# microsoft/fadtk

Hardware: NVIDIA H100
Metric: audio_seconds_embedded_per_second (higher is better)
Workload: dtype f16

## Files before the change

fadtk_b200/csrc/conv_gemm.cuh:

```cuda
#pragma once
#include "sm90.cuh"

namespace fad {

struct ConvGemmParams {
    int taps;
    int cblks;
    int box_w, box_h, box_n;
    int tiles_w, tiles_h;
    int img_groups;
    int n_tiles;
    int H, W, NB, Cout;
    int lo_adds;
    int ld_out, n_valid;
    int relu, pool;
    const float* bias;
    __half* out;
    float* out_f32;
    float* resid;
    int resid_C, resid_res, resid_shift;
};

__device__ __forceinline__ long long window_row_to_token(long long o, int res, int shift) {
    const int lg_nw = 28 - __clz(res);
// ... 2 lines not shown
    const long long wi = o >> 6;
    const int wx = (int)wi & (nw - 1);
    const int wy = (int)(wi >> lg_nw) & (nw - 1);
    const long long b = wi >> (2 * lg_nw);
    int y = wy * 8 + (in >> 3) + shift, xx = wx * 8 + (in & 7) + shift;
    if (y >= res) y -= res;
    if (xx >= res) xx -= res;
    return (b * res + y) * res + xx;
}

constexpr int kTileM = 128;
constexpr int kBlockK = 64;
constexpr int kConvGemmThreads = 512;
constexpr int kConsumers = 2;
constexpr int kConsumerRegs = 168;
constexpr int kEpiRegs = 136;
constexpr int kClusterCtas = 2;
constexpr int kChunkSteps = 8;
constexpr float kAccumShrinkPerElement = 1.06e-9f;
constexpr uint32_t kABytes = kTileM * kBlockK * 2;
constexpr uint32_t kEpiRowBytes = 128 * 4;
constexpr uint32_t kEpiBytes = 64 * kEpiRowBytes;
constexpr uint32_t kBiasBytes = 128 * 4;
static_assert(40 + kEpiRegs + kConsumers * kConsumerRegs <= 65536 / 128, "register file over-subscribed");
static_assert(kConsumerRegs > 65536 / kConvGemmThreads, "the consumers raise their register count (setmaxnreg.inc)");

template <int N_TILE, int WMODE>
__host__ __device__ constexpr uint32_t conv_gemm_stage_bytes() {
    return kABytes + (WMODE == 1 ? 2 : 1) * N_TILE * kBlockK * 2;
}

template <int N_TILE, int STAGES, int WMODE>
__host__ __device__ constexpr uint32_t conv_gemm_smem_bytes() {
    return STAGES * conv_gemm_stage_bytes<N_TILE, WMODE>() + 1024  + 256
         + kConsumers * kEpiBytes + 4 * kBiasBytes;
}

__device__ __forceinline__ uint32_t pack_half2(float a, float b) {
    __half2 h = __floats2half2_rn(a, b);
    return *reinterpret_cast<uint32_t*>(&h);
}
template <int N>
__device__ __forceinline__ void gelu_erf_n(float* x) {
    float z[N], q[N];
#pragma unroll
    for (int i = 0; i < N; ++i) { z[i] = fminf(fabsf(x[i]) * 0.70710678118654752f, 4.3f); q[i] = 1.04899843e-04f; }
    constexpr float kQ[6] = {-4.92790774e-04f, -2.22368206e-03f, 2.93586859e-02f, -1.48908889e-01f, -9.18342944e-01f,
                             -1.62791250e+00f};
#pragma unroll
    for (int t = 0; t < 6; ++t) {
#pragma unroll
        for (int i = 0; i < N; ++i) q[i] = fmaf(q[i], z[i], kQ[t]);
    }
#pragma unroll
    for (int i = 0; i < N; ++i) asm("ex2.approx.ftz.f32 %0, %1;" : "=f"(q[i]) : "f"(q[i] * z[i]));
#pragma unroll
    for (int i = 0; i < N; ++i) x[i] = 0.5f * x[i] * (1.0f + copysignf(1.0f - q[i], x[i]));
}
__device__ __forceinline__ float gelu_erf(float x) {
    gelu_erf_n<1>(&x);
    return x;
}

template <int N>
__device__ __forceinline__ void elu_ex2_n(float* x) {
    float e[N], t[N];
#pragma unroll
    for (int i = 0; i < N; ++i) asm("ex2.approx.ftz.f32 %0, %1;" : "=f"(e[i]) : "f"(fminf(x[i], 0.f) * 1.4426950408889634f));
#pragma unroll
    for (int i = 0; i < N; ++i) t[i] = x[i] * fmaf(x[i], fmaf(x[i], fmaf(x[i], 4.16666667e-2f, 1.66666667e-1f), 0.5f), 1.0f);
#pragma unroll
    for (int i = 0; i < N; ++i) x[i] = x[i] > 0.f ? x[i] : (x[i] > -0.0625f ? t[i] : e[i] - 1.0f);
}

__device__ __forceinline__ uint32_t hmax2_u32(uint32_t a, uint32_t b) {
    __half2 r = __hmax2(*reinterpret_cast<__half2*>(&a), *reinterpret_cast<__half2*>(&b));
    return *reinterpret_cast<uint32_t*>(&r);
}

template <int N_TILE, int STAGES, int WMODE>
__global__ void __launch_bounds__(kConvGemmThreads, 1)
conv_gemm_kernel(const __grid_constant__ CUtensorMap map_x,
                 const __grid_constant__ CUtensorMap map_w,
                 const ConvGemmParams p)
{
    using namespace sm90;
    static_assert(N_TILE == 128, "one m64n128 accumulator per consumer warpgroup");
    static_assert(WMODE == 0 || WMODE == 1, "WMODE 0: fp16 weights, 1: fp16 hi/lo pair");
    static_assert(kClusterCtas == 2, "the work units below are M-tile pairs");
    constexpr bool SPLIT_W = WMODE == 1;
    constexpr uint32_t kStageBytes = conv_gemm_stage_bytes<N_TILE, WMODE>();
    constexpr int kBRows = (SPLIT_W ? 2 : 1) * N_TILE;
    constexpr int kGroups = N_TILE / 32;

    extern __shared__ uint8_t smem_raw[];
    uint8_t* smem = reinterpret_cast<uint8_t*>((reinterpret_cast<uintptr_t>(smem_raw) + 1023) & ~uintptr_t(1023));
    uint64_t* bars = reinterpret_cast<uint64_t*>(smem + STAGES * kStageBytes);
    uint64_t* full = bars;
    uint64_t* empty = bars + STAGES;
    uint64_t* epi_full = bars + 2 * STAGES;
    uint64_t* epi_empty = bars + 2 * STAGES + kConsumers;
    static_assert((2 * STAGES + 2 * kConsumers) * 8 <= 256, "barriers");
    uint8_t* epi = smem + STAGES * kStageBytes + 256;

    const int warp = threadIdx.x >> 5;
    const int lane = threadIdx.x & 31;
    const int ksteps = p.taps * p.cblks;
    const int n_chunks = (ksteps + kChunkSteps - 1) / kChunkSteps;
    const int chunk_len = (ksteps + n_chunks - 1) / n_chunks;
    const int m_tiles = p.img_groups * p.tiles_h * p.tiles_w;
    const int n_clusters = (int)gridDim.x / kClusterCtas;
    const int total_units = (m_tiles + 1) / 2 * p.n_tiles;

    if (warp == 0 && lane == 0) {
        tma_prefetch_desc(&map_x);
        tma_prefetch_desc(&map_w);
    }
    if (warp == 1 && lane == 0) {
        for (int s = 0; s < STAGES; ++s) { mbar_init(&full[s], 1); mbar_init(&empty[s], kClusterCtas * kConsumers * 4); }
        for (int c = 0; c < kConsumers; ++c) { mbar_init(&epi_full[c], 128); mbar_init(&epi_empty[c], 64); }
        mbar_fence_init();
    }
    cluster_sync();

    if (warp < 4) {
        setmaxnreg_dec<40>();
        if (warp == 0 && elect_one()) {
            const int rank = (int)cluster_ctarank();
            const int cluster = (int)cluster_index();
            constexpr int kHalfRows = kBRows / kClusterCtas;
            uint8_t* const w_half = smem + kABytes + rank * kHalfRows * 128;
            int s = 0; uint32_t ph = 0;
            for (int unit = cluster; unit < total_units; unit += n_clusters) {
                const int nt = unit % p.n_tiles;
                const int m = min(2 * (unit / p.n_tiles) + rank, m_tiles - 1);
                const int w0 = (m % p.tiles_w) * p.box_w;
                const int h0 = ((m / p.tiles_w) % p.tiles_h) * p.box_h;
                const int n0 = (m / (p.tiles_w * p.tiles_h)) * p.box_n;
                for (int ks = 0; ks < ksteps; ++ks) {
                    const int tap = ks / p.cblks;
                    const int cb = ks - tap * p.cblks;
                    int dh = 0, dw = 0;
                    if (p.taps == 9) { dh = tap / 3 - 1; dw = tap % 3 - 1; }
                    mbar_wait(&empty[s], ph ^ 1);
                    uint8_t* st = smem + s * kStageBytes;
                    mbar_expect_tx(&full[s], kStageBytes);
                    tma_load_4d(st, &map_x, &full[s], cb * kBlockK, w0 + dw, h0 + dh, n0);
                    tma_load_2d_multicast(w_half + s * kStageBytes, &map_w, &full[s], ks * kBlockK,
                                          nt * kBRows + rank * kHalfRows, (1u << kClusterCtas) - 1);
                    if (++s == STAGES) { s = 0; ph ^= 1; }
                }
            }
        }
    } else if (warp < 4 + 4 * kConsumers) {
        setmaxnreg_inc<kConsumerRegs>();
        const int cluster = (int)cluster_index();
        const int c = (warp >> 2) - 1;
        const int wq = warp & 3;
        const uint32_t epi_base = smem_u32(epi) + c * kEpiBytes;
        int s = 0; uint32_t ph = 0, eph = 0;
        auto release = [&](int st_) {
            __syncwarp();
            if (lane == 0) {
#pragma unroll
                for (int cta = 0; cta < kClusterCtas; ++cta) mbar_arrive_cluster(&empty[st_], cta);
            }
        };

        for (int unit = cluster; unit < total_units; unit += n_clusters) {
            float sum[64], acc[64];
#pragma unroll
            for (int i = 0; i < 64; ++i) sum[i] = 0.f;
            for (int ks0 = 0; ks0 < ksteps; ks0 += chunk_len) {
                const int ks1 = min(ks0 + chunk_len, ksteps);
                const float unshrink = kAccumShrinkPerElement * (float)((ks1 - ks0) * kBlockK * (SPLIT_W && p.lo_adds ? 2 : 1));
                int prev_s = -1;
                for (int ks = ks0; ks < ks1; ++ks) {
                    mbar_wait(&full[s], ph);
                    const uint32_t a_addr = smem_u32(smem + s * kStageBytes);
                    const uint64_t a_desc = kmajor_sw128_desc(a_addr + c * 64 * 128);
                    const uint64_t b_desc = kmajor_sw128_desc(a_addr + kABytes);
                    wgmma_fence();
#pragma unroll
                    for (int k = 0; k < kBlockK / 16; ++k) {
                        wgmma_m64n128k16_f16<0, 0>(acc, a_desc + 2 * k, b_desc + 2 * k, (ks > ks0) || (k > 0));
                        if (SPLIT_W)
                            wgmma_m64n128k16_f16<0, 0>(acc, a_desc + 2 * k, b_desc + 2 * k + (N_TILE * 128 / 16), 1);
                    }
                    wgmma_commit();
                    wgmma_wait<1>();
                    if (prev_s >= 0) release(prev_s);
                    prev_s = s;
                    if (++s == STAGES) { s = 0; ph ^= 1; }
                }
                wgmma_wait<0>();
                fence_regs(acc);
                release(prev_s);
#pragma unroll
                for (int i = 0; i < 64; ++i) sum[i] += fmaf(acc[i], unshrink, acc[i]);
            }

            mbar_wait(&epi_empty[c], eph ^ 1);
            const int fr = wq * 16 + (lane >> 2);
            const uint32_t x = ((lane & 3) >> 1) ^ (fr & 7);
            const uint32_t row_base = epi_base + fr * kEpiRowBytes + (lane & 1) * 8;
#pragma unroll
            for (int jl = 0; jl < 4; ++jl) {
                const uint32_t a = row_base + (((2 * jl) ^ x) << 4);
#pragma unroll
                for (int jh = 0; jh < 4; ++jh) {
#pragma unroll
                    for (int i = 0; i < 2; ++i) {
                        const int j = 4 * jh + jl;
                        sts64(a + i * 8 * kEpiRowBytes + jh * 128, sum[4 * j + 2 * i], sum[4 * j + 2 * i + 1]);
                    }
                }
            }
            mbar_arrive(&epi_full[c]);
            eph ^= 1;
        }
    } else {
        if constexpr (kEpiRegs > 65536 / kConvGemmThreads) setmaxnreg_inc<kEpiRegs>();
        else setmaxnreg_dec<kEpiRegs>();
        const int rank = (int)cluster_ctarank();
        const int cluster = (int)cluster_index();
        const int e = warp - 4 - 4 * kConsumers;
        const int c = e >> 1;
        const int rr = (e & 1) * 32 + lane;
        const int r = c * 64 + rr;
        const int bw = p.box_w, bh = p.box_h;
        const int pw = r % bw;
        const int phh = (r / bw) % bh;
        const int pn = r / (bw * bh);
        const uint32_t wrows = smem_u32(epi) + c * kEpiBytes + (e & 1) * 32 * kEpiRowBytes;
        const uint32_t row_mine = wrows + lane * kEpiRowBytes;
        const uint32_t bias_s = smem_u32(epi) + kConsumers * kEpiBytes + e * kBiasBytes;
        const int sw = lane & 7;
        const int cq = lane & 7, rq = lane >> 3;
        uint32_t eph = 0;
        const bool plain = p.tiles_w == 1 && p.tiles_h == 1 && bw == 1 && bh == 1;
        const bool f32_path = p.out_f32 != nullptr || p.resid != nullptr;
        auto prefetch_resid = [&](int nt_, int m_) {
            if (p.resid == nullptr || !plain) return;
            const int n_ = m_ * kTileM + r;
            if (n_ >= p.NB) return;
            const long long tok = p.resid_res ? window_row_to_token((long long)n_, p.resid_res, p.resid_shift) : (long long)n_;
            for (int cc = nt_ * N_TILE; cc < nt_ * N_TILE + N_TILE && cc < p.resid_C; cc += 32)
                asm volatile("prefetch.global.L2 [%0];" :: "l"(p.resid + tok * p.resid_C + cc));
        };
        if (cluster < total_units) prefetch_resid(cluster % p.n_tiles, 2 * (cluster / p.n_tiles) + rank);

        for (int unit = cluster; unit < total_units; unit += n_clusters) {
            const int nt = unit % p.n_tiles;
            const int m = 2 * (unit / p.n_tiles) + rank;
            if (unit + n_clusters < total_units)
                prefetch_resid((unit + n_clusters) % p.n_tiles, 2 * ((unit + n_clusters) / p.n_tiles) + rank);
            __syncwarp();
            {
                const float4 b = __ldg(reinterpret_cast<const float4*>(p.bias + nt * N_TILE) + lane);
                sts128(bias_s + lane * 16, __float_as_uint(b.x), __float_as_uint(b.y), __float_as_uint(b.z), __float_as_uint(b.w));
            }
            __syncwarp();

            int w, h, n;
            if (plain) { w = 0; h = 0; n = m * kTileM + r; }
            else {
                w = (m % p.tiles_w) * bw + pw;
                h = ((m / p.tiles_w) % p.tiles_h) * bh + phh;
                n = (m / (p.tiles_w * p.tiles_h)) * p.box_n + pn;
            }
            const bool valid = n < p.NB;
            const int ch0 = nt * N_TILE;
            long long out_off = -1, res_off = -1;
            if (valid && !p.pool) {
                out_off = (long long)((size_t(n) * p.H + h) * p.W + w) * p.ld_out;
                if (p.resid != nullptr)
                    res_off = (p.resid_res ? window_row_to_token((long long)n, p.resid_res, p.resid_shift) : (long long)n)
                              * p.resid_C;
            }

            mbar_wait(&epi_full[c], eph);
#pragma unroll 1
            for (int g = 0; g < kGroups; ++g) {
                float f[32];
#pragma unroll
                for (int j = 0; j < 8; ++j) {
                    const uint4 u = lds128(row_mine + g * 128 + ((j ^ sw) << 4));
                    const uint4 b = lds128(bias_s + g * 128 + j * 16);
                    f[4 * j + 0] = __uint_as_float(u.x) + __uint_as_float(b.x);
                    f[4 * j + 1] = __uint_as_float(u.y) + __uint_as_float(b.y);
                    f[4 * j + 2] = __uint_as_float(u.z) + __uint_as_float(b.z);
                    f[4 * j + 3] = __uint_as_float(u.w) + __uint_as_float(b.w);
                }
                if (p.relu == 1) {
#pragma unroll
                    for (int j = 0; j < 32; ++j) f[j] = fmaxf(f[j], 0.0f);
                } else if (p.relu == 2) {
#pragma unroll
                    for (int j = 0; j < 32; j += 8) gelu_erf_n<8>(f + j);
                } else if (p.relu == 3) {
#pragma unroll
                    for (int j = 0; j < 32; j += 8) elu_ex2_n<8>(f + j);
                }

                if (!p.pool) {
                    if (f32_path) {
                        if (p.out != nullptr && out_off >= 0) {
                            uint4* dst = reinterpret_cast<uint4*>(p.out + out_off + ch0 + g * 32);
#pragma unroll
                            for (int j = 0; j < 4; ++j)
                                if (ch0 + g * 32 + 8 * j < p.n_valid)
                                    dst[j] = make_uint4(pack_half2(f[8 * j], f[8 * j + 1]), pack_half2(f[8 * j + 2], f[8 * j + 3]),
                                                        pack_half2(f[8 * j + 4], f[8 * j + 5]), pack_half2(f[8 * j + 6], f[8 * j + 7]));
                        }
#pragma unroll
                        for (int j = 0; j < 8; ++j)
                            sts128(row_mine + g * 128 + ((j ^ sw) << 4), __float_as_uint(f[4 * j]), __float_as_uint(f[4 * j + 1]),
                                   __float_as_uint(f[4 * j + 2]), __float_as_uint(f[4 * j + 3]));
                        __syncwarp();
                        const int col = ch0 + g * 32 + cq * 4;
#pragma unroll
                        for (int hf = 0; hf < 2; ++hf) {
                            float4 v[4];
#pragma unroll
                            for (int it = 0; it < 4; ++it) {
                                const int x = (hf * 4 + it) * 4 + rq;
                                const uint4 u = lds128(wrows + x * kEpiRowBytes + g * 128 + ((cq ^ (x & 7)) << 4));
                                v[it] = make_float4(__uint_as_float(u.x), __uint_as_float(u.y), __uint_as_float(u.z), __uint_as_float(u.w));
                            }
                            if (p.out_f32 != nullptr) {
#pragma unroll
                                for (int it = 0; it < 4; ++it) {
                                    const long long off = __shfl_sync(0xffffffffu, out_off, (hf * 4 + it) * 4 + rq);
                                    if (off >= 0 && col < p.n_valid) *reinterpret_cast<float4*>(p.out_f32 + off + col) = v[it];
                                }
                            }
                            if (p.resid != nullptr && ch0 + g * 32 < p.resid_C) {
                                long long offs[4];
                                float4 xv[4];
#pragma unroll
                                for (int it = 0; it < 4; ++it) {
                                    offs[it] = __shfl_sync(0xffffffffu, res_off, (hf * 4 + it) * 4 + rq);
                                    if (offs[it] >= 0) xv[it] = *reinterpret_cast<const float4*>(p.resid + offs[it] + col);
                                }
#pragma unroll
                                for (int it = 0; it < 4; ++it) {
                                    if (offs[it] >= 0) {
                                        const float4 a = v[it];
                                        xv[it].x += a.x; xv[it].y += a.y; xv[it].z += a.z; xv[it].w += a.w;
                                        *reinterpret_cast<float4*>(p.resid + offs[it] + col) = xv[it];
                                    }
                                }
                            }
                        }
                    } else if (p.out != nullptr) {
                        const int seg = (g & ~1) * 128;
#pragma unroll
                        for (int j = 0; j < 4; ++j)
                            sts128(row_mine + seg + ((((g & 1) * 4 + j) ^ sw) << 4),
                                   pack_half2(f[8 * j], f[8 * j + 1]), pack_half2(f[8 * j + 2], f[8 * j + 3]),
                                   pack_half2(f[8 * j + 4], f[8 * j + 5]), pack_half2(f[8 * j + 6], f[8 * j + 7]));
                        if (g & 1) {
                            __syncwarp();
                            const int col = ch0 + (g - 1) * 32 + cq * 8;
#pragma unroll
                            for (int it = 0; it < 8; ++it) {
                                const int x = it * 4 + rq;
                                const uint4 v = lds128(wrows + x * kEpiRowBytes + seg + ((cq ^ (x & 7)) << 4));
                                const long long off = __shfl_sync(0xffffffffu, out_off, x);
                                if (off >= 0 && col < p.n_valid) *reinterpret_cast<uint4*>(p.out + off + col) = v;
                            }
                        }
                    }
                } else {
                    uint32_t h2[16];
#pragma unroll
                    for (int j = 0; j < 16; ++j) h2[j] = pack_half2(f[2 * j], f[2 * j + 1]);
#pragma unroll
                    for (int j = 0; j < 16; ++j) {
                        uint32_t o = __shfl_xor_sync(0xffffffffu, h2[j], 1);
                        h2[j] = hmax2_u32(h2[j], o);
                        o = __shfl_xor_sync(0xffffffffu, h2[j], bw);
                        h2[j] = hmax2_u32(h2[j], o);
                    }
                    const int sub = (pw & 1) | ((phh & 1) << 1);
                    uint4 o;
                    o.x = sub == 0 ? h2[0] : sub == 1 ? h2[4] : sub == 2 ? h2[8]  : h2[12];
                    o.y = sub == 0 ? h2[1] : sub == 1 ? h2[5] : sub == 2 ? h2[9]  : h2[13];
                    o.z = sub == 0 ? h2[2] : sub == 1 ? h2[6] : sub == 2 ? h2[10] : h2[14];
                    o.w = sub == 0 ? h2[3] : sub == 1 ? h2[7] : sub == 2 ? h2[11] : h2[15];
                    if (valid) {
                        const size_t pix = (size_t(n) * (p.H >> 1) + (h >> 1)) * (p.W >> 1) + (w >> 1);
                        *reinterpret_cast<uint4*>(p.out + pix * p.Cout + ch0 + g * 32 + sub * 8) = o;
                    }
                }
            }
            mbar_arrive(&epi_empty[c]);
            eph ^= 1;
        }
    }
    cluster_sync();
}

}
```

fadtk_b200/csrc/fadtk_b200.cu:

```cuda
#include "../../include/fadtk_b200.h"

#include <cuda.h>
#include <cuda_runtime.h>
#include <cuda_fp16.h>
#include <cxxabi.h>
#include <algorithm>
#include <cmath>
#include <cstdio>
#include <cstdlib>
#include <cstring>
#include <initializer_list>
#include <memory>
#include <set>
#include <string>
#include <type_traits>
#include <utility>
#include <vector>

#include "conv_gemm.cuh"
#include "frontend.cuh"
#include "stats.cuh"
#include "frechet.cuh"
#include "clap.cuh"
#include "resample.cuh"
// ... 132 lines not shown
        while (bh * 2 <= 128 / g.box_w && H % (bh * 2) == 0) bh *= 2;
        g.box_h = bh;
        g.box_n = 128 / (g.box_w * g.box_h);
    }
    if (pool && (g.box_h % 2 != 0 || g.box_w % 2 != 0)) return fail("pooling needs even tile boxes");
    if (Cout % 128 != 0) return fail("Cout must be a multiple of 128");
    g.n_tile = 128;
    return 0;
}

struct VggState;
struct ClapState;
struct WhisperState;
struct EncodecState;
struct W2vState;

}

struct fad_handle {
    int device = 0;
    int num_sms = 0;
    int max_examples = 0;
    long long launches = 0;
    int gemm_clusters[2] = {};

    std::vector<DeviceBuffer> mem;
    double *d_twiddle = nullptr, *d_hann = nullptr, *d_melw = nullptr;
    int *d_mel_start = nullptr, *d_mel_count = nullptr;

    DeviceBuffer ws_tiles, ws_sums, gather_buf;
    DeviceBuffer fr_buf;
    DeviceBuffer rs_bank, rs_mono;
    int rs_in = 0, rs_out = 0;
    DeviceBuffer pair_buf;
    DeviceBuffer agree_buf;
    std::set<const void*> zero_lo;

    void* nccl_comm = nullptr;

    std::unique_ptr<VggState> vgg;
    std::unique_ptr<ClapState> clap;
    std::unique_ptr<WhisperState> whisper;
    std::unique_ptr<EncodecState> encodec;
    std::unique_ptr<W2vState> w2v;
    ~fad_handle();

    bool prof_on = false;
// ... 20 lines not shown
template <typename... Params, typename... Args>
int launch_attrs(fad_handle* h, void (*kernel)(Params...), dim3 grid, dim3 block, size_t smem, cudaStream_t st,
                 cudaLaunchAttribute* attrs, unsigned n_attrs, Args&&... args) {
    if (grid.x == 0 || grid.y == 0 || grid.z == 0) return 0;
    cudaLaunchConfig_t cfg = {};
    cfg.gridDim = grid;
    cfg.blockDim = block;
    cfg.dynamicSmemBytes = smem;
    cfg.stream = st;
    cfg.attrs = attrs;
    cfg.numAttrs = n_attrs;
    cudaError_t e = cudaLaunchKernelEx(&cfg, kernel, std::forward<Args>(args)...);
    const cudaError_t last = cudaGetLastError();
    if (e == cudaSuccess) e = last;
    if (e != cudaSuccess) return fail(kernel_name((const void*)kernel) + ": " + cudaGetErrorString(e));
    h->launches++;
    return 0;
}
template <typename... Params, typename... Args>
int launch(fad_handle* h, void (*kernel)(Params...), dim3 grid, dim3 block, size_t smem, cudaStream_t st, Args&&... args) {
    return launch_attrs(h, kernel, grid, block, smem, st, nullptr, 0, std::forward<Args>(args)...);
}

template <int WMODE> struct Gemm {
    static constexpr int kStages = WMODE ? 3 : 4;
    static constexpr uint32_t kSmem = fad::conv_gemm_smem_bytes<128, kStages, WMODE>();
    static_assert(kSmem <= 227 * 1024, "over the per-CTA shared-memory limit");
    static constexpr auto kernel = fad::conv_gemm_kernel<128, kStages, WMODE>;
};

cudaLaunchAttribute cta_pair() {
    cudaLaunchAttribute attr = {};
    attr.id = cudaLaunchAttributeClusterDimension;
    attr.val.clusterDim.x = fad::kClusterCtas; attr.val.clusterDim.y = 1; attr.val.clusterDim.z = 1;
    return attr;
}

template <int WMODE>
int setup_gemm(fad_handle* h) {
    CK(cudaFuncSetAttribute(Gemm<WMODE>::kernel, cudaFuncAttributeMaxDynamicSharedMemorySize, (int)Gemm<WMODE>::kSmem));
    cudaLaunchAttribute attr = cta_pair();
    cudaLaunchConfig_t cfg = {};
    cfg.gridDim = dim3(fad::kClusterCtas * (unsigned)h->num_sms);
    cfg.blockDim = dim3(fad::kConvGemmThreads);
    cfg.dynamicSmemBytes = Gemm<WMODE>::kSmem;
    cfg.attrs = &attr;
    cfg.numAttrs = 1;
    CK(cudaOccupancyMaxActiveClusters(&h->gemm_clusters[WMODE], Gemm<WMODE>::kernel, &cfg));
    if (h->gemm_clusters[WMODE] <= 0) return fail("conv_gemm_kernel: no CTA pair fits on the device");
    return 0;
}

template <int WMODE>
int launch_conv_gemm(fad_handle* h, const CUtensorMap& mx, const CUtensorMap& mw, const fad::ConvGemmParams& p, cudaStream_t st) {
    const int units = (p.img_groups * p.tiles_h * p.tiles_w + 1) / 2 * p.n_tiles;
    cudaLaunchAttribute attr = cta_pair();
    return launch_attrs(h, Gemm<WMODE>::kernel, dim3(fad::kClusterCtas * (unsigned)std::min(units, h->gemm_clusters[WMODE])),
                        dim3(fad::kConvGemmThreads), Gemm<WMODE>::kSmem, st, &attr, 1, mx, mw, p);
}

int encode_layer_maps(const LayerGeom& g, const void* x, long long nb_dim, const void* w,
                      CUtensorMap* mx, CUtensorMap* mw, int a_cols = 0, long long a_row_stride = 0) {
    const uint64_t ac = a_cols > 0 ? (uint64_t)a_cols : (uint64_t)g.Cin;
    const uint64_t xd[4] = {ac, (uint64_t)g.W, (uint64_t)g.H, (uint64_t)nb_dim};
    uint64_t xs[3] = {ac * 2, (uint64_t)g.W * ac * 2, (uint64_t)g.H * g.W * ac * 2};
    if (a_row_stride > 0) xs[0] = xs[1] = xs[2] = (uint64_t)a_row_stride * 2;
    const uint32_t xb[4] = {64, (uint32_t)g.box_w, (uint32_t)g.box_h, (uint32_t)g.box_n};
    if (encode_f16_map(mx, x, 4, xd, xs, xb)) return 1;
    const uint64_t K = (uint64_t)g.taps * g.Cin;
    const uint64_t rows_mul = g.split_w ? 2 : 1;
    const uint64_t wd[2] = {K, (uint64_t)g.Cout * rows_mul};
    const uint64_t ws[1] = {K * 2};
    const uint32_t wb[2] = {64, (uint32_t)(g.n_tile * rows_mul / fad::kClusterCtas)};
    return encode_f16_map(mw, w, 2, wd, ws, wb);
}

int launch_attention_wgmma(fad_handle* h, const __half* qkv, long long n_clips, int S, int d, int heads, __half* out, cudaStream_t st) {
    if (heads * 64 != d) return fail("attention_wgmma: head dimension must be 64");
    CUtensorMap map;
    const uint64_t dims[3] = {(uint64_t)3 * d, (uint64_t)S, (uint64_t)n_clips};
    const uint64_t strides[2] = {(uint64_t)3 * d * 2, (uint64_t)S * 3 * d * 2};
// ... 1 lines not shown
    if (encode_f16_map(&map, qkv, 3, dims, strides, box)) return 1;
    fad::AttnParams p;
    p.S = S; p.d = d; p.heads = heads; p.out = out;
    return launch(h, fad::attention_wgmma_kernel, dim3((S + 127) / 128, heads, (unsigned)n_clips), fad::kAtThreads, fad::kAtSmem,
                  st, map, p);
}

int run_layer(fad_handle* h, const LayerGeom& g, const CUtensorMap& mx, const CUtensorMap& mw, const void* w,
              int NB, const float* bias, void* out, float* out_f32, cudaStream_t st,
              float* resid = nullptr, int resid_C = 0, int resid_res = 0, int resid_shift = 0, int n_valid = 0) {
    fad::ConvGemmParams p;
    p.taps = g.taps; p.cblks = g.Cin / 64;
    p.box_w = g.box_w; p.box_h = g.box_h; p.box_n = g.box_n;
    p.tiles_w = g.W / g.box_w; p.tiles_h = g.H / g.box_h;
    p.img_groups = (NB + g.box_n - 1) / g.box_n;
    p.n_tiles = g.Cout / g.n_tile;
    p.H = g.H; p.W = g.W; p.NB = NB; p.Cout = g.Cout;
    p.n_valid = n_valid > 0 ? n_valid : g.Cout;
    p.ld_out = p.n_valid;
    p.relu = g.relu; p.pool = g.pool;
    p.bias = bias; p.out = reinterpret_cast<__half*>(out); p.out_f32 = out_f32;
    p.resid = resid; p.resid_C = resid_C; p.resid_res = resid_res; p.resid_shift = resid_shift;
    p.lo_adds = g.split_w == 1 && h->zero_lo.count(w) == 0;
    if (g.split_w) return launch_conv_gemm<1>(h, mx, mw, p, st);
    return launch_conv_gemm<0>(h, mx, mw, p, st);
}

__global__ void wlo_absmax_kernel(const __half* __restrict__ w, long long n_tiles, long long K, unsigned int* __restrict__ out) {
    float m = 0.f;
    const long long total = n_tiles * 128 * K;
    for (long long e = blockIdx.x * (long long)blockDim.x + threadIdx.x; e < total; e += (long long)gridDim.x * blockDim.x) {
        const long long row = e / K, k = e - row * K;
        const long long t = row >> 7, j = row & 127;
        m = fmaxf(m, fabsf(__half2float(w[((t * 256 + 128 + j) * K) + k])));
    }
    for (int o = 16; o > 0; o >>= 1) m = fmaxf(m, __shfl_xor_sync(0xffffffffu, m, o));
    if ((threadIdx.x & 31) == 0) atomicMax(out, __float_as_uint(m));
}
int note_split_weights(fad_handle* h, const void* w, long long n_tiles, long long K, cudaStream_t st) {
    DeviceBuffer d_max;
    if (d_max.grow(4)) return 1;
    unsigned int mx = 0;
    const unsigned blocks = (unsigned)std::max<long long>(1, std::min<long long>((n_tiles * 128 * K + 255) / 256, (long long)h->num_sms * 16));
    CK(cudaMemsetAsync(d_max.get(), 0, 4, st));
    if (launch(h, wlo_absmax_kernel, blocks, 256, 0, st, reinterpret_cast<const __half*>(w), n_tiles, K, d_max.get<unsigned int>()))
        return 1;
    CK(cudaMemcpyAsync(&mx, d_max.get(), 4, cudaMemcpyDeviceToHost, st));
    CK(cudaStreamSynchronize(st));
// ... 155 lines not shown
        upload(h->mem, &h->d_melw, melw.data(), melw.size() * 8) || upload(h->mem, &h->d_mel_start, ms.data(), ms.size() * 4) ||
        upload(h->mem, &h->d_mel_count, mc.data(), mc.size() * 4)) return 1;
    const auto smem = [](const void* kernel, size_t bytes) {
        return cudaFuncSetAttribute(kernel, cudaFuncAttributeMaxDynamicSharedMemorySize, (int)bytes);
    };
    CK(smem((const void*)fad::logmel_kernel<double>, fad::logmel_smem_bytes<double>()));
    CK(smem((const void*)fad::logmel_kernel<float>, fad::logmel_smem_bytes<float>()));
    CK(smem((const void*)fad::clap_logmel_kernel, fad::clap_logmel_smem_bytes()));
    CK(smem((const void*)fad::attention_wgmma_kernel, fad::kAtSmem));
    CK(smem((const void*)fad::clap_window_attention_kernel<24>, fad::att_smem_bytes(24, fad::kAttWarps, fad::kAttStages)));
    CK(smem((const void*)fad::clap_window_attention_kernel<32>, fad::att_smem_bytes(32, fad::kAttWarps, fad::kAttStages)));
    CK(smem((const void*)fad::kad_tile_kernel<0>, fad::kKadSmemBytes));
    CK(smem((const void*)fad::kad_tile_kernel<1>, fad::kKadSmemBytes));
    CK(smem((const void*)fad::kad_tile_kernel<2>, fad::kKadSmemBytes));
    CK(smem((const void*)fad::kad_perm_tile_kernel<false>, fad::kPermSmemBytes));
    CK(smem((const void*)fad::kad_perm_tile_kernel<true>, fad::kPermSmemBytes));
    CK(smem((const void*)fad::prdc_tile_kernel<0>, fad::kPairSmemBytes));
    CK(smem((const void*)fad::prdc_tile_kernel<1>, fad::kPairSmemBytes));
    CK(smem((const void*)fad::prdc_tile_kernel<2>, fad::kPairSmemBytes));
    CK(smem((const void*)fad::prdc_tile_kernel<3>, fad::kPrdcSongSmemBytes));
    CK(smem((const void*)fad::prdc_tile_kernel<4>, fad::kPairSmemBytes));
    CK(smem((const void*)fad::prdc_tile_kernel<5>, fad::kPrdcNearestSmemBytes));
    CK(smem((const void*)fad::prdc_tile_kernel<6>, fad::kPairSmemBytes));
    if (setup_gemm<0>(h.get()) || setup_gemm<1>(h.get())) return 1;
    *out = h.release();
    return 0;
}

int fad_destroy(fad_handle* h) {
    if (!h) return 0;
    cudaSetDevice(h->device);
    fad_comm_destroy(h);
    delete h;
    return 0;
}

long long fad_launch_count(fad_handle* h) { return h ? h->launches : 0; }

int fad_vggish_load(fad_handle* h, const fad_vggish_weights* w) {
    if (!h || !w) return fail("null argument");
    const void* src[18] = {w->conv1_w_host, w->conv1_b_host,
                           w->conv_w_host[0], w->conv_w_host[1], w->conv_w_host[2], w->conv_w_host[3], w->conv_w_host[4],
                           w->fc_w_host[0], w->fc_w_host[1], w->fc_w_host[2],
                           w->conv_b_host[0], w->conv_b_host[1], w->conv_b_host[2], w->conv_b_host[3], w->conv_b_host[4],
                           w->fc_b_host[0], w->fc_b_host[1], w->fc_b_host[2]};
    if (check_tensors("fad_vggish_load", src, 18)) return 1;
    const void* const* wsrc = src + 2;
// ... 525 lines not shown
```

fadtk_b200/csrc/sm90.cuh:

```cuda
#pragma once
#include <cuda.h>
#include <cuda_fp16.h>
#include <stdint.h>
#include <stdio.h>

namespace sm90 {

__device__ __forceinline__ uint32_t smem_u32(const void* p) {
    return static_cast<uint32_t>(__cvta_generic_to_shared(p));
}
__device__ __forceinline__ uint32_t lane_id() { return threadIdx.x & 31; }

__device__ __forceinline__ bool elect_one() {
    uint32_t pred;
    asm volatile(
        "{\n\t.reg .pred P;\n\t"
        "elect.sync _|P, 0xffffffff;\n\t"
        "selp.u32 %0, 1, 0, P;\n\t}\n"
        : "=r"(pred));
    return pred != 0;
}

template <uint32_t kRegs> __device__ __forceinline__ void setmaxnreg_inc() {
    asm volatile("setmaxnreg.inc.sync.aligned.u32 %0;" ::"n"(kRegs));
}
template <uint32_t kRegs> __device__ __forceinline__ void setmaxnreg_dec() {
    asm volatile("setmaxnreg.dec.sync.aligned.u32 %0;" ::"n"(kRegs));
}

__device__ __forceinline__ void named_bar_sync(uint32_t id, uint32_t count) {
    asm volatile("bar.sync %0, %1;" ::"r"(id), "r"(count) : "memory");
}

__device__ __forceinline__ void sts128(uint32_t addr, uint32_t x, uint32_t y, uint32_t z, uint32_t w) {
    asm volatile("st.shared.v4.b32 [%0], {%1, %2, %3, %4};" ::"r"(addr), "r"(x), "r"(y), "r"(z), "r"(w) : "memory");
}
__device__ __forceinline__ uint4 lds128(uint32_t addr) {
    uint4 v;
    asm volatile("ld.shared.v4.b32 {%0, %1, %2, %3}, [%4];" : "=r"(v.x), "=r"(v.y), "=r"(v.z), "=r"(v.w) : "r"(addr) : "memory");
    return v;
}
__device__ __forceinline__ void sts64(uint32_t addr, float x, float y) {
    asm volatile("st.shared.v2.f32 [%0], {%1, %2};" ::"r"(addr), "f"(x), "f"(y) : "memory");
}

__device__ __forceinline__ void dmma_884(double& c0, double& c1, double a, double b) {
    asm volatile("mma.sync.aligned.m8n8k4.row.col.f64.f64.f64.f64 {%0, %1}, {%2}, {%3}, {%0, %1};"
                 : "+d"(c0), "+d"(c1) : "d"(a), "d"(b));
}

__device__ __forceinline__ void mbar_init(uint64_t* bar, uint32_t count) {
    asm volatile("mbarrier.init.shared::cta.b64 [%0], %1;" ::"r"(smem_u32(bar)), "r"(count));
}
__device__ __forceinline__ void mbar_fence_init() {
    asm volatile("fence.mbarrier_init.release.cluster;" ::: "memory");
}
__device__ __forceinline__ void mbar_expect_tx(uint64_t* bar, uint32_t bytes) {
    asm volatile("mbarrier.arrive.expect_tx.shared::cta.b64 _, [%0], %1;"
                 ::"r"(smem_u32(bar)), "r"(bytes) : "memory");
}
__device__ __forceinline__ void mbar_arrive(uint64_t* bar) {
    asm volatile("mbarrier.arrive.shared::cta.b64 _, [%0];" ::"r"(smem_u32(bar)) : "memory");
}
__device__ __forceinline__ bool mbar_try_wait(uint64_t* bar, uint32_t parity) {
    uint32_t ok;
    asm volatile(
// ... 166 lines not shown
```

Baseline: 178,300.

## Add fp16 epilogue tile path with stmatrix staging and extra pipeline stages

Measured after the change: 183,300 (median of 6 runs). 1.03x the previous value.

```diff
diff --git a/fadtk_b200/csrc/conv_gemm.cuh b/fadtk_b200/csrc/conv_gemm.cuh
--- a/fadtk_b200/csrc/conv_gemm.cuh
+++ b/fadtk_b200/csrc/conv_gemm.cuh
@@ -48,6 +48,9 @@
 constexpr uint32_t kEpiRowBytes = 128 * 4;
 constexpr uint32_t kEpiBytes = 64 * kEpiRowBytes;
 constexpr uint32_t kBiasBytes = 128 * 4;
+constexpr uint32_t kEpiRowBytesF16 = 128 * 2;
+constexpr uint32_t kEpiBytesF16 = 64 * kEpiRowBytesF16;
+constexpr uint32_t kMaxSmemPerCta = 227 * 1024;
 static_assert(40 + kEpiRegs + kConsumers * kConsumerRegs <= 65536 / 128, "register file over-subscribed");
 static_assert(kConsumerRegs > 65536 / kConvGemmThreads, "the consumers raise their register count (setmaxnreg.inc)");
 
@@ -56,10 +59,15 @@
     return kABytes + (WMODE == 1 ? 2 : 1) * N_TILE * kBlockK * 2;
 }
 
-template <int N_TILE, int STAGES, int WMODE>
+template <int N_TILE, int STAGES, int WMODE, bool F16_TILE>
 __host__ __device__ constexpr uint32_t conv_gemm_smem_bytes() {
     return STAGES * conv_gemm_stage_bytes<N_TILE, WMODE>() + 1024  + 256
-         + kConsumers * kEpiBytes + 4 * kBiasBytes;
+         + (F16_TILE ? kConsumers * (kEpiBytesF16 + kBiasBytes) : kConsumers * kEpiBytes + 4 * kBiasBytes);
+}
+
+template <int N_TILE, int WMODE, bool F16_TILE>
+__host__ __device__ constexpr int conv_gemm_max_stages() {
+    return (int)((kMaxSmemPerCta - conv_gemm_smem_bytes<N_TILE, 0, WMODE, F16_TILE>()) / conv_gemm_stage_bytes<N_TILE, WMODE>());
 }
 
 __device__ __forceinline__ uint32_t pack_half2(float a, float b) {
@@ -104,7 +112,7 @@
     return *reinterpret_cast<uint32_t*>(&r);
 }
 
-template <int N_TILE, int STAGES, int WMODE>
+template <int N_TILE, int STAGES, int WMODE, bool F16_TILE>
 __global__ void __launch_bounds__(kConvGemmThreads, 1)
 conv_gemm_kernel(const __grid_constant__ CUtensorMap map_x,
                  const __grid_constant__ CUtensorMap map_w,
@@ -114,6 +122,7 @@
     static_assert(N_TILE == 128, "one m64n128 accumulator per consumer warpgroup");
     static_assert(WMODE == 0 || WMODE == 1, "WMODE 0: fp16 weights, 1: fp16 hi/lo pair");
     static_assert(kClusterCtas == 2, "the work units below are M-tile pairs");
+    static_assert(conv_gemm_smem_bytes<N_TILE, STAGES, WMODE, F16_TILE>() <= kMaxSmemPerCta, "stages do not fit");
     constexpr bool SPLIT_W = WMODE == 1;
     constexpr uint32_t kStageBytes = conv_gemm_stage_bytes<N_TILE, WMODE>();
     constexpr int kBRows = (SPLIT_W ? 2 : 1) * N_TILE;
@@ -128,6 +137,7 @@
     uint64_t* epi_empty = bars + 2 * STAGES + kConsumers;
     static_assert((2 * STAGES + 2 * kConsumers) * 8 <= 256, "barriers");
     uint8_t* epi = smem + STAGES * kStageBytes + 256;
+    float* const bias_f16 = reinterpret_cast<float*>(epi + kConsumers * kEpiBytesF16);
 
     const int warp = threadIdx.x >> 5;
     const int lane = threadIdx.x & 31;
@@ -146,6 +156,11 @@
         for (int s = 0; s < STAGES; ++s) { mbar_init(&full[s], 1); mbar_init(&empty[s], kClusterCtas * kConsumers * 4); }
         for (int c = 0; c < kConsumers; ++c) { mbar_init(&epi_full[c], 128); mbar_init(&epi_empty[c], 64); }
         mbar_fence_init();
+    }
+    if constexpr (F16_TILE) {
+        const int first = (int)cluster_index();
+        if (first < total_units && threadIdx.x < kConsumers * N_TILE)
+            bias_f16[threadIdx.x] = p.bias[(first % p.n_tiles) * N_TILE + threadIdx.x % N_TILE];
     }
     cluster_sync();
 
@@ -183,7 +198,7 @@
         const int cluster = (int)cluster_index();
         const int c = (warp >> 2) - 1;
         const int wq = warp & 3;
-        const uint32_t epi_base = smem_u32(epi) + c * kEpiBytes;
+        const uint32_t epi_base = smem_u32(epi) + c * (F16_TILE ? kEpiBytesF16 : kEpiBytes);
         int s = 0; uint32_t ph = 0, eph = 0;
         auto release = [&](int st_) {
             __syncwarp();
@@ -224,6 +239,39 @@
                 release(prev_s);
 #pragma unroll
                 for (int i = 0; i < 64; ++i) sum[i] += fmaf(acc[i], unshrink, acc[i]);
+            }
+
+            if constexpr (F16_TILE) {
+                mbar_wait(&epi_empty[c], eph ^ 1);
+                const uint32_t bias_s = smem_u32(bias_f16) + c * kBiasBytes + 8 * (lane & 3);
+                uint32_t h2[32];
+#pragma unroll
+                for (int j0 = 0; j0 < 16; j0 += 8) {
+                    float2 b[8];
+#pragma unroll
+                    for (int j = 0; j < 8; ++j) b[j] = lds64(bias_s + 32 * (j0 + j));
+#pragma unroll
+                    for (int jj = 0; jj < 8; ++jj) {
+                        const int j = j0 + jj;
+                        float v[4] = {sum[4 * j] + b[jj].x, sum[4 * j + 1] + b[jj].y, sum[4 * j + 2] + b[jj].x,
+                                      sum[4 * j + 3] + b[jj].y};
+                        if (p.relu == 1) {
+#pragma unroll
+                            for (int t = 0; t < 4; ++t) v[t] = fmaxf(v[t], 0.0f);
+                        }
+                        h2[2 * j] = pack_half2(v[0], v[1]);
+                        h2[2 * j + 1] = pack_half2(v[2], v[3]);
+                    }
+                }
+                const int mi = lane >> 3;
+                const uint32_t row_addr = epi_base + (wq * 16 + (mi & 1) * 8 + (lane & 7)) * kEpiRowBytesF16;
+#pragma unroll
+                for (int j = 0; j < 16; j += 2)
+                    stmatrix_x4(row_addr + (((j + (mi >> 1)) ^ (lane & 7)) << 4), h2[2 * j], h2[2 * j + 1], h2[2 * j + 2],
+                                h2[2 * j + 3]);
+                mbar_arrive(&epi_full[c]);
+                eph ^= 1;
+                continue;
             }
 
             mbar_wait(&epi_empty[c], eph ^ 1);
@@ -258,8 +306,9 @@
         const int pw = r % bw;
         const int phh = (r / bw) % bh;
         const int pn = r / (bw * bh);
-        const uint32_t wrows = smem_u32(epi) + c * kEpiBytes + (e & 1) * 32 * kEpiRowBytes;
-        const uint32_t row_mine = wrows + lane * kEpiRowBytes;
+        constexpr uint32_t kRowBytes = F16_TILE ? kEpiRowBytesF16 : kEpiRowBytes;
+        const uint32_t wrows = smem_u32(epi) + c * (F16_TILE ? kEpiBytesF16 : kEpiBytes) + (e & 1) * 32 * kRowBytes;
+        const uint32_t row_mine = wrows + lane * kRowBytes;
         const uint32_t bias_s = smem_u32(epi) + kConsumers * kEpiBytes + e * kBiasBytes;
         const int sw = lane & 7;
         const int cq = lane & 7, rq = lane >> 3;
@@ -281,12 +330,14 @@
             const int m = 2 * (unit / p.n_tiles) + rank;
             if (unit + n_clusters < total_units)
                 prefetch_resid((unit + n_clusters) % p.n_tiles, 2 * ((unit + n_clusters) / p.n_tiles) + rank);
-            __syncwarp();
-            {
-                const float4 b = __ldg(reinterpret_cast<const float4*>(p.bias + nt * N_TILE) + lane);
-                sts128(bias_s + lane * 16, __float_as_uint(b.x), __float_as_uint(b.y), __float_as_uint(b.z), __float_as_uint(b.w));
-            }
-            __syncwarp();
+            if constexpr (!F16_TILE) {
+                __syncwarp();
+                {
+                    const float4 b = __ldg(reinterpret_cast<const float4*>(p.bias + nt * N_TILE) + lane);
+                    sts128(bias_s + lane * 16, __float_as_uint(b.x), __float_as_uint(b.y), __float_as_uint(b.z), __float_as_uint(b.w));
+                }
+                __syncwarp();
+            }
 
             int w, h, n;
             if (plain) { w = 0; h = 0; n = m * kTileM + r; }
@@ -305,120 +356,156 @@
                               * p.resid_C;
             }
 
+            auto pool_store = [&](uint32_t (&h2)[16], int g) {
+#pragma unroll
+                for (int j = 0; j < 16; ++j) {
+                    uint32_t o = __shfl_xor_sync(0xffffffffu, h2[j], 1);
+                    h2[j] = hmax2_u32(h2[j], o);
+                    o = __shfl_xor_sync(0xffffffffu, h2[j], bw);
+                    h2[j] = hmax2_u32(h2[j], o);
+                }
+                const int sub = (pw & 1) | ((phh & 1) << 1);
+                uint4 o;
+                o.x = sub == 0 ? h2[0] : sub == 1 ? h2[4] : sub == 2 ? h2[8]  : h2[12];
+                o.y = sub == 0 ? h2[1] : sub == 1 ? h2[5] : sub == 2 ? h2[9]  : h2[13];
+                o.z = sub == 0 ? h2[2] : sub == 1 ? h2[6] : sub == 2 ? h2[10] : h2[14];
+                o.w = sub == 0 ? h2[3] : sub == 1 ? h2[7] : sub == 2 ? h2[11] : h2[15];
+                if (valid) {
+                    const size_t pix = (size_t(n) * (p.H >> 1) + (h >> 1)) * (p.W >> 1) + (w >> 1);
+                    *reinterpret_cast<uint4*>(p.out + pix * p.Cout + ch0 + g * 32 + sub * 8) = o;
+                }
+            };
+
             mbar_wait(&epi_full[c], eph);
+            if constexpr (F16_TILE) {
+                if (p.pool) {
 #pragma unroll 1
-            for (int g = 0; g < kGroups; ++g) {
-                float f[32];
-#pragma unroll
-                for (int j = 0; j < 8; ++j) {
-                    const uint4 u = lds128(row_mine + g * 128 + ((j ^ sw) << 4));
-                    const uint4 b = lds128(bias_s + g * 128 + j * 16);
-                    f[4 * j + 0] = __uint_as_float(u.x) + __uint_as_float(b.x);
-                    f[4 * j + 1] = __uint_as_float(u.y) + __uint_as_float(b.y);
-                    f[4 * j + 2] = __uint_as_float(u.z) + __uint_as_float(b.z);
-                    f[4 * j + 3] = __uint_as_float(u.w) + __uint_as_float(b.w);
-                }
-                if (p.relu == 1) {
-#pragma unroll
-                    for (int j = 0; j < 32; ++j) f[j] = fmaxf(f[j], 0.0f);
-                } else if (p.relu == 2) {
-#pragma unroll
-                    for (int j = 0; j < 32; j += 8) gelu_erf_n<8>(f + j);
-                } else if (p.relu == 3) {
-#pragma unroll
-                    for (int j = 0; j < 32; j += 8) elu_ex2_n<8>(f + j);
-                }
-
-                if (!p.pool) {
-                    if (f32_path) {
-                        if (p.out != nullptr && out_off >= 0) {
-                            uint4* dst = reinterpret_cast<uint4*>(p.out + out_off + ch0 + g * 32);
-#pragma unroll
-                            for (int j = 0; j < 4; ++j)
-                                if (ch0 + g * 32 + 8 * j < p.n_valid)
-                                    dst[j] = make_uint4(pack_half2(f[8 * j], f[8 * j + 1]), pack_half2(f[8 * j + 2], f[8 * j + 3]),
-                                                        pack_half2(f[8 * j + 4], f[8 * j + 5]), pack_half2(f[8 * j + 6], f[8 * j + 7]));
+                    for (int g = 0; g < kGroups; ++g) {
+                        uint32_t h2[16];
+#pragma unroll
+                        for (int j = 0; j < 4; ++j) {
+                            const uint4 u = lds128(row_mine + (((4 * g + j) ^ sw) << 4));
+                            h2[4 * j] = u.x; h2[4 * j + 1] = u.y; h2[4 * j + 2] = u.z; h2[4 * j + 3] = u.w;
                         }
-#pragma unroll
-                        for (int j = 0; j < 8; ++j)
-                            sts128(row_mine + g * 128 + ((j ^ sw) << 4), __float_as_uint(f[4 * j]), __float_as_uint(f[4 * j + 1]),
-                                   __float_as_uint(f[4 * j + 2]), __float_as_uint(f[4 * j + 3]));
-                        __syncwarp();
-                        const int col = ch0 + g * 32 + cq * 4;
-#pragma unroll
-                        for (int hf = 0; hf < 2; ++hf) {
-                            float4 v[4];
-#pragma unroll
-                            for (int it = 0; it < 4; ++it) {
-                                const int x = (hf * 4 + it) * 4 + rq;
-                                const uint4 u = lds128(wrows + x * kEpiRowBytes + g * 128 + ((cq ^ (x & 7)) << 4));
-                                v[it] = make_float4(__uint_as_float(u.x), __uint_as_float(u.y), __uint_as_float(u.z), __uint_as_float(u.w));
+                        pool_store(h2, g);
+                    }
+                } else {
+                    const int fq = lane & 15, frq = lane >> 4;
+                    const int col = ch0 + fq * 8;
+#pragma unroll 8
+                    for (int it = 0; it < 16; ++it) {
+                        const int x = 2 * it + frq;
+                        const uint4 v = lds128(wrows + x * kRowBytes + ((fq ^ (x & 7)) << 4));
+                        const long long off = __shfl_sync(0xffffffffu, out_off, x);
+                        if (off >= 0 && col < p.n_valid) *reinterpret_cast<uint4*>(p.out + off + col) = v;
+                    }
+                }
+            } else {
+#pragma unroll 1
+                for (int g = 0; g < kGroups; ++g) {
+                    float f[32];
+#pragma unroll
+                    for (int j = 0; j < 8; ++j) {
+                        const uint4 u = lds128(row_mine + g * 128 + ((j ^ sw) << 4));
+                        const uint4 b = lds128(bias_s + g * 128 + j * 16);
+                        f[4 * j + 0] = __uint_as_float(u.x) + __uint_as_float(b.x);
+                        f[4 * j + 1] = __uint_as_float(u.y) + __uint_as_float(b.y);
+                        f[4 * j + 2] = __uint_as_float(u.z) + __uint_as_float(b.z);
+                        f[4 * j + 3] = __uint_as_float(u.w) + __uint_as_float(b.w);
+                    }
+                    if (p.relu == 1) {
+#pragma unroll
+                        for (int j = 0; j < 32; ++j) f[j] = fmaxf(f[j], 0.0f);
+                    } else if (p.relu == 2) {
+#pragma unroll
+                        for (int j = 0; j < 32; j += 8) gelu_erf_n<8>(f + j);
+                    } else if (p.relu == 3) {
+#pragma unroll
+                        for (int j = 0; j < 32; j += 8) elu_ex2_n<8>(f + j);
+                    }
+
+                    if (!p.pool) {
+                        if (f32_path) {
+                            if (p.out != nullptr && out_off >= 0) {
+                                uint4* dst = reinterpret_cast<uint4*>(p.out + out_off + ch0 + g * 32);
+#pragma unroll
+                                for (int j = 0; j < 4; ++j)
+                                    if (ch0 + g * 32 + 8 * j < p.n_valid)
+                                        dst[j] = make_uint4(pack_half2(f[8 * j], f[8 * j + 1]), pack_half2(f[8 * j + 2], f[8 * j + 3]),
+                                                            pack_half2(f[8 * j + 4], f[8 * j + 5]), pack_half2(f[8 * j + 6], f[8 * j + 7]));
                             }
-                            if (p.out_f32 != nullptr) {
+#pragma unroll
+                            for (int j = 0; j < 8; ++j)
+                                sts128(row_mine + g * 128 + ((j ^ sw) << 4), __float_as_uint(f[4 * j]), __float_as_uint(f[4 * j + 1]),
+                                       __float_as_uint(f[4 * j + 2]), __float_as_uint(f[4 * j + 3]));
+                            __syncwarp();
+                            const int col = ch0 + g * 32 + cq * 4;
+#pragma unroll
+                            for (int hf = 0; hf < 2; ++hf) {
+                                float4 v[4];
 #pragma unroll
                                 for (int it = 0; it < 4; ++it) {
-                                    const long long off = __shfl_sync(0xffffffffu, out_off, (hf * 4 + it) * 4 + rq);
-                                    if (off >= 0 && col < p.n_valid) *reinterpret_cast<float4*>(p.out_f32 + off + col) = v[it];
+                                    const int x = (hf * 4 + it) * 4 + rq;
+                                    const uint4 u = lds128(wrows + x * kEpiRowBytes + g * 128 + ((cq ^ (x & 7)) << 4));
+                                    v[it] = make_float4(__uint_as_float(u.x), __uint_as_float(u.y), __uint_as_float(u.z), __uint_as_float(u.w));
                                 }
-                            }
-                            if (p.resid != nullptr && ch0 + g * 32 < p.resid_C) {
-                                long long offs[4];
-                                float4 xv[4];
-#pragma unroll
-                                for (int it = 0; it < 4; ++it) {
-                                    offs[it] = __shfl_sync(0xffffffffu, res_off, (hf * 4 + it) * 4 + rq);
-                                    if (offs[it] >= 0) xv[it] = *reinterpret_cast<const float4*>(p.resid + offs[it] + col);
+                                if (p.out_f32 != nullptr) {
+#pragma unroll
+                                    for (int it = 0; it < 4; ++it) {
+                                        const long long off = __shfl_sync(0xffffffffu, out_off, (hf * 4 + it) * 4 + rq);
+                                        if (off >= 0 && col < p.n_valid) *reinterpret_cast<float4*>(p.out_f32 + off + col) = v[it];
+                                    }
                                 }
-#pragma unroll
-                                for (int it = 0; it < 4; ++it) {
-                                    if (offs[it] >= 0) {
-                                        const float4 a = v[it];
-                                        xv[it].x += a.x; xv[it].y += a.y; xv[it].z += a.z; xv[it].w += a.w;
-                                        *reinterpret_cast<float4*>(p.resid + offs[it] + col) = xv[it];
+                                if (p.resid != nullptr && ch0 + g * 32 < p.resid_C) {
+                                    long long offs[4];
+                                    float4 xv[4];
+#pragma unroll
+                                    for (int it = 0; it < 4; ++it) {
+                                        offs[it] = __shfl_sync(0xffffffffu, res_off, (hf * 4 + it) * 4 + rq);
+                                        if (offs[it] >= 0) xv[it] = *reinterpret_cast<const float4*>(p.resid + offs[it] + col);
+                                    }
+#pragma unroll
+                                    for (int it = 0; it < 4; ++it) {
+                                        if (offs[it] >= 0) {
+                                            const float4 a = v[it];
+                                            xv[it].x += a.x; xv[it].y += a.y; xv[it].z += a.z; xv[it].w += a.w;
+                                            *reinterpret_cast<float4*>(p.resid + offs[it] + col) = xv[it];
+                                        }
                                     }
                                 }
                             }
-                        }
-                    } else if (p.out != nullptr) {
-                        const int seg = (g & ~1) * 128;
-#pragma unroll
-                        for (int j = 0; j < 4; ++j)
-                            sts128(row_mine + seg + ((((g & 1) * 4 + j) ^ sw) << 4),
-                                   pack_half2(f[8 * j], f[8 * j + 1]), pack_half2(f[8 * j + 2], f[8 * j + 3]),
-                                   pack_half2(f[8 * j + 4], f[8 * j + 5]), pack_half2(f[8 * j + 6], f[8 * j + 7]));
-                        if (g & 1) {
-                            __syncwarp();
-                            const int col = ch0 + (g - 1) * 32 + cq * 8;
-#pragma unroll
-                            for (int it = 0; it < 8; ++it) {
-                                const int x = it * 4 + rq;
-                                const uint4 v = lds128(wrows + x * kEpiRowBytes + seg + ((cq ^ (x & 7)) << 4));
-                                const long long off = __shfl_sync(0xffffffffu, out_off, x);
-                                if (off >= 0 && col < p.n_valid) *reinterpret_cast<uint4*>(p.out + off + col) = v;
+                        } else if (p.out != nullptr) {
+                            const int seg = (g & ~1) * 128;
+#pragma unroll
+                            for (int j = 0; j < 4; ++j)
+                                sts128(row_mine + seg + ((((g & 1) * 4 + j) ^ sw) << 4),
+                                       pack_half2(f[8 * j], f[8 * j + 1]), pack_half2(f[8 * j + 2], f[8 * j + 3]),
+                                       pack_half2(f[8 * j + 4], f[8 * j + 5]), pack_half2(f[8 * j + 6], f[8 * j + 7]));
+                            if (g & 1) {
+                                __syncwarp();
+                                const int col = ch0 + (g - 1) * 32 + cq * 8;
+#pragma unroll
+                                for (int it = 0; it < 8; ++it) {
+                                    const int x = it * 4 + rq;
+                                    const uint4 v = lds128(wrows + x * kEpiRowBytes + seg + ((cq ^ (x & 7)) << 4));
+                                    const long long off = __shfl_sync(0xffffffffu, out_off, x);
+                                    if (off >= 0 && col < p.n_valid) *reinterpret_cast<uint4*>(p.out + off + col) = v;
+                                }
                             }
                         }
-                    }
-                } else {
-                    uint32_t h2[16];
-#pragma unroll
-                    for (int j = 0; j < 16; ++j) h2[j] = pack_half2(f[2 * j], f[2 * j + 1]);
-#pragma unroll
-                    for (int j = 0; j < 16; ++j) {
-                        uint32_t o = __shfl_xor_sync(0xffffffffu, h2[j], 1);
-                        h2[j] = hmax2_u32(h2[j], o);
-                        o = __shfl_xor_sync(0xffffffffu, h2[j], bw);
-                        h2[j] = hmax2_u32(h2[j], o);
-                    }
-                    const int sub = (pw & 1) | ((phh & 1) << 1);
-                    uint4 o;
-                    o.x = sub == 0 ? h2[0] : sub == 1 ? h2[4] : sub == 2 ? h2[8]  : h2[12];
-                    o.y = sub == 0 ? h2[1] : sub == 1 ? h2[5] : sub == 2 ? h2[9]  : h2[13];
-                    o.z = sub == 0 ? h2[2] : sub == 1 ? h2[6] : sub == 2 ? h2[10] : h2[14];
-                    o.w = sub == 0 ? h2[3] : sub == 1 ? h2[7] : sub == 2 ? h2[11] : h2[15];
-                    if (valid) {
-                        const size_t pix = (size_t(n) * (p.H >> 1) + (h >> 1)) * (p.W >> 1) + (w >> 1);
-                        *reinterpret_cast<uint4*>(p.out + pix * p.Cout + ch0 + g * 32 + sub * 8) = o;
-                    }
+                    } else {
+                        uint32_t h2[16];
+#pragma unroll
+                        for (int j = 0; j < 16; ++j) h2[j] = pack_half2(f[2 * j], f[2 * j + 1]);
+                        pool_store(h2, g);
+                    }
+                }
+            }
+            if constexpr (F16_TILE) {
+                if ((e & 1) == 0 && unit + n_clusters < total_units) {
+                    const float4 b = __ldg(reinterpret_cast<const float4*>(p.bias + ((unit + n_clusters) % p.n_tiles) * N_TILE) + lane);
+                    sts128(smem_u32(bias_f16) + c * kBiasBytes + lane * 16, __float_as_uint(b.x), __float_as_uint(b.y),
+                           __float_as_uint(b.z), __float_as_uint(b.w));
                 }
             }
             mbar_arrive(&epi_empty[c]);
diff --git a/fadtk_b200/csrc/fadtk_b200.cu b/fadtk_b200/csrc/fadtk_b200.cu
--- a/fadtk_b200/csrc/fadtk_b200.cu
+++ b/fadtk_b200/csrc/fadtk_b200.cu
@@ -178,7 +178,7 @@
     int num_sms = 0;
     int max_examples = 0;
     long long launches = 0;
-    int gemm_clusters[2] = {};
+    int gemm_clusters[2][2] = {};
 
     std::vector<DeviceBuffer> mem;
     double *d_twiddle = nullptr, *d_hann = nullptr, *d_melw = nullptr;
@@ -245,11 +245,10 @@
     return launch_attrs(h, kernel, grid, block, smem, st, nullptr, 0, std::forward<Args>(args)...);
 }
 
-template <int WMODE> struct Gemm {
-    static constexpr int kStages = WMODE ? 3 : 4;
-    static constexpr uint32_t kSmem = fad::conv_gemm_smem_bytes<128, kStages, WMODE>();
-    static_assert(kSmem <= 227 * 1024, "over the per-CTA shared-memory limit");
-    static constexpr auto kernel = fad::conv_gemm_kernel<128, kStages, WMODE>;
+template <int WMODE, bool F16_TILE> struct Gemm {
+    static constexpr int kStages = fad::conv_gemm_max_stages<128, WMODE, F16_TILE>();
+    static constexpr uint32_t kSmem = fad::conv_gemm_smem_bytes<128, kStages, WMODE, F16_TILE>();
+    static constexpr auto kernel = fad::conv_gemm_kernel<128, kStages, WMODE, F16_TILE>;
 };
 
 cudaLaunchAttribute cta_pair() {
@@ -259,27 +258,29 @@
     return attr;
 }
 
-template <int WMODE>
+template <int WMODE, bool F16_TILE>
 int setup_gemm(fad_handle* h) {
-    CK(cudaFuncSetAttribute(Gemm<WMODE>::kernel, cudaFuncAttributeMaxDynamicSharedMemorySize, (int)Gemm<WMODE>::kSmem));
+    using G = Gemm<WMODE, F16_TILE>;
+    CK(cudaFuncSetAttribute(G::kernel, cudaFuncAttributeMaxDynamicSharedMemorySize, (int)G::kSmem));
     cudaLaunchAttribute attr = cta_pair();
     cudaLaunchConfig_t cfg = {};
     cfg.gridDim = dim3(fad::kClusterCtas * (unsigned)h->num_sms);
     cfg.blockDim = dim3(fad::kConvGemmThreads);
-    cfg.dynamicSmemBytes = Gemm<WMODE>::kSmem;
+    cfg.dynamicSmemBytes = G::kSmem;
     cfg.attrs = &attr;
     cfg.numAttrs = 1;
-    CK(cudaOccupancyMaxActiveClusters(&h->gemm_clusters[WMODE], Gemm<WMODE>::kernel, &cfg));
-    if (h->gemm_clusters[WMODE] <= 0) return fail("conv_gemm_kernel: no CTA pair fits on the device");
-    return 0;
-}
-
-template <int WMODE>
+    CK(cudaOccupancyMaxActiveClusters(&h->gemm_clusters[WMODE][F16_TILE], G::kernel, &cfg));
+    if (h->gemm_clusters[WMODE][F16_TILE] <= 0) return fail("conv_gemm_kernel: no CTA pair fits on the device");
+    return 0;
+}
+
+template <int WMODE, bool F16_TILE>
 int launch_conv_gemm(fad_handle* h, const CUtensorMap& mx, const CUtensorMap& mw, const fad::ConvGemmParams& p, cudaStream_t st) {
+    using G = Gemm<WMODE, F16_TILE>;
     const int units = (p.img_groups * p.tiles_h * p.tiles_w + 1) / 2 * p.n_tiles;
     cudaLaunchAttribute attr = cta_pair();
-    return launch_attrs(h, Gemm<WMODE>::kernel, dim3(fad::kClusterCtas * (unsigned)std::min(units, h->gemm_clusters[WMODE])),
-                        dim3(fad::kConvGemmThreads), Gemm<WMODE>::kSmem, st, &attr, 1, mx, mw, p);
+    return launch_attrs(h, G::kernel, dim3(fad::kClusterCtas * (unsigned)std::min(units, h->gemm_clusters[WMODE][F16_TILE])),
+                        dim3(fad::kConvGemmThreads), G::kSmem, st, &attr, 1, mx, mw, p);
 }
 
 int encode_layer_maps(const LayerGeom& g, const void* x, long long nb_dim, const void* w,
@@ -327,8 +328,9 @@
     p.bias = bias; p.out = reinterpret_cast<__half*>(out); p.out_f32 = out_f32;
     p.resid = resid; p.resid_C = resid_C; p.resid_res = resid_res; p.resid_shift = resid_shift;
     p.lo_adds = g.split_w == 1 && h->zero_lo.count(w) == 0;
-    if (g.split_w) return launch_conv_gemm<1>(h, mx, mw, p, st);
-    return launch_conv_gemm<0>(h, mx, mw, p, st);
+    const bool f16_tile = out != nullptr && out_f32 == nullptr && resid == nullptr && (g.relu == 0 || g.relu == 1);
+    if (g.split_w) return f16_tile ? launch_conv_gemm<1, true>(h, mx, mw, p, st) : launch_conv_gemm<1, false>(h, mx, mw, p, st);
+    return f16_tile ? launch_conv_gemm<0, true>(h, mx, mw, p, st) : launch_conv_gemm<0, false>(h, mx, mw, p, st);
 }
 
 __global__ void wlo_absmax_kernel(const __half* __restrict__ w, long long n_tiles, long long K, unsigned int* __restrict__ out) {
@@ -530,7 +532,8 @@
     CK(smem((const void*)fad::prdc_tile_kernel<4>, fad::kPairSmemBytes));
     CK(smem((const void*)fad::prdc_tile_kernel<5>, fad::kPrdcNearestSmemBytes));
     CK(smem((const void*)fad::prdc_tile_kernel<6>, fad::kPairSmemBytes));
-    if (setup_gemm<0>(h.get()) || setup_gemm<1>(h.get())) return 1;
+    if (setup_gemm<0, false>(h.get()) || setup_gemm<1, false>(h.get()) || setup_gemm<0, true>(h.get()) ||
+        setup_gemm<1, true>(h.get())) return 1;
     *out = h.release();
     return 0;
 }
diff --git a/fadtk_b200/csrc/sm90.cuh b/fadtk_b200/csrc/sm90.cuh
--- a/fadtk_b200/csrc/sm90.cuh
+++ b/fadtk_b200/csrc/sm90.cuh
@@ -40,8 +40,17 @@
     asm volatile("ld.shared.v4.b32 {%0, %1, %2, %3}, [%4];" : "=r"(v.x), "=r"(v.y), "=r"(v.z), "=r"(v.w) : "r"(addr) : "memory");
     return v;
 }
+__device__ __forceinline__ float2 lds64(uint32_t addr) {
+    float2 v;
+    asm volatile("ld.shared.v2.f32 {%0, %1}, [%2];" : "=f"(v.x), "=f"(v.y) : "r"(addr) : "memory");
+    return v;
+}
 __device__ __forceinline__ void sts64(uint32_t addr, float x, float y) {
     asm volatile("st.shared.v2.f32 [%0], {%1, %2};" ::"r"(addr), "f"(x), "f"(y) : "memory");
+}
+__device__ __forceinline__ void stmatrix_x4(uint32_t addr, uint32_t r0, uint32_t r1, uint32_t r2, uint32_t r3) {
+    asm volatile("stmatrix.sync.aligned.m8n8.x4.shared.b16 [%0], {%1, %2, %3, %4};"
+                 ::"r"(addr), "r"(r0), "r"(r1), "r"(r2), "r"(r3) : "memory");
 }
 
 __device__ __forceinline__ void dmma_884(double& c0, double& c1, double a, double b) {
```
